# OpenRL-Lab/openrl

Measured on AMD Instinct MI355X. Metric: env-steps/sec (collect+PPO update), 4096-env CartPole-shape, higher is better.
Workload: dtype f32

## Files before the change

### openrl_amd/csrc/orl_mlp.h

```cpp
#pragma once
#include "orl_common.h"

namespace orl {

typedef float f32x4 __attribute__((ext_vector_type(4)));

constexpr int HID = 64;
constexpr int W2S = 68;
constexpr int TILE_B = 16;

#define ORL_MFMA(a, b, c) __builtin_amdgcn_mfma_f32_16x16x4f32((a), (b), (c), 0, 0, 0)
#ifdef ORL_SPLIT_PROBE
#define ORL_IF_FULL(x)
#else
#define ORL_IF_FULL(x) x
#endif

typedef unsigned u32x4 __attribute__((ext_vector_type(4)));
typedef __bf16 bf16x8 __attribute__((ext_vector_type(8)));
typedef float f32x16 __attribute__((ext_vector_type(16)));

#ifndef ORL_WBS
#define ORL_WBS 80
#endif
// ... 244 lines not shown
  return __builtin_bit_cast(unsigned, __builtin_convertvector(f32x2{a, b}, f16x2));
}
__device__ __forceinline__ float rem16_lo(unsigned pk, float x) {
  float r;
  asm("v_fma_mix_f32 %0, %1, -1.0, %2 op_sel_hi:[1,0,0]" : "=v"(r) : "v"(pk), "v"(x));
  return r;
}
__device__ __forceinline__ float rem16_hi(unsigned pk, float x) {
  float r;
  asm("v_fma_mix_f32 %0, %1, -1.0, %2 op_sel:[1,0,0] op_sel_hi:[1,0,0]" : "=v"(r) : "v"(pk), "v"(x));
  return r;
}
__device__ __forceinline__ void split8h(const float (&x)[8], u32x4& hi, u32x4& lo) {
#pragma unroll
  for (int p = 0; p < 4; ++p) {
    const float a = x[2 * p], b = x[2 * p + 1];
    hi[p] = cvt_pk_f16(a, b);
    lo[p] = cvt_pk_f16(rem16_lo(hi[p], a), rem16_hi(hi[p], b));
  }
}
__device__ __forceinline__ f32x4 mfma_f16_16(u32x4 a, u32x4 b, f32x4 c) {
  return __builtin_amdgcn_mfma_f32_16x16x32_f16(__builtin_bit_cast(f16x8, a), __builtin_bit_cast(f16x8, b), c, 0, 0, 0);
}
__device__ __forceinline__ f32x16 mfma_f16_32(u32x4 a, u32x4 b, f32x16 c) {
  return __builtin_amdgcn_mfma_f32_32x32x16_f16(__builtin_bit_cast(f16x8, a), __builtin_bit_cast(f16x8, b), c, 0, 0, 0);
}
__device__ __forceinline__ void split_weight_store2h(unsigned short* __restrict__ img, int o, int k, float w0, float w1) {
  const int m = k >> 4, q = (k >> 2) & 3, r = k & 3, h = m >> 1, sl = (m & 1) * 4 + r;
  const unsigned hi = cvt_pk_f16(w0, w1);
  *(unsigned*)(img + wb_off(0, o, h, q) + sl) = hi;
  *(unsigned*)(img + wb_off(1, o, h, q) + sl) = cvt_pk_f16(rem16_lo(hi, w0), rem16_hi(hi, w1));
}
__device__ __forceinline__ void split_Th(const f32x4 (&in)[4], u32x4 (&xs)[2][2]) {
#pragma unroll
  for (int h = 0; h < 2; ++h) {
    float x[8];
#pragma unroll
    for (int r = 0; r < 4; ++r) { x[r] = in[2 * h][r]; x[4 + r] = in[2 * h + 1][r]; }
    split8h(x, xs[h][0], xs[h][1]);
  }
}
__device__ __forceinline__ void mm64_T_h2(const unsigned short* __restrict__ Wb, const u32x4 (&xs)[2][2], f32x4 (&acc)[4], int j,
                                          int q) {
  u32x4 w[2][2];
#pragma unroll
  for (int p = 0; p < 2; ++p) w[0][p] = *(const u32x4*)(Wb + wb_off(p, j, 0, q));
#pragma unroll
  for (int st = 0; st < 8; ++st) {
    const int h = st >> 2, mo = st & 3;
    if (st < 7) {
      const int h2 = (st + 1) >> 2, mo2 = (st + 1) & 3;
#pragma unroll
      for (int p = 0; p < 2; ++p) w[(st + 1) & 1][p] = *(const u32x4*)(Wb + wb_off(p, 16 * mo2 + j, h2, q));
    }
    const u32x4 wh = w[st & 1][0], wl = w[st & 1][1];
    acc[mo] = mfma_f16_16(wl, xs[h][0], acc[mo]);
    acc[mo] = mfma_f16_16(wh, xs[h][1], acc[mo]);
    acc[mo] = mfma_f16_16(wh, xs[h][0], acc[mo]);
  }
}
__device__ __forceinline__ void mm64_T_h2_tr(const unsigned short* __restrict__ Wb, const u32x4 (&xs)[2][2], f32x4 (&acc)[4],
                                             int j, int q) {
  const unsigned short* base = Wb + (4 * q + (j >> 2)) * WBS + (j & 3) * 8;
  auto frag = [&](int p, int h, int mo) -> u32x4 {
    const unsigned short* a = base + (p * HID + 32 * h) * WBS + (mo >> 1) * 32 + (mo & 1) * 4;
    const u32x2 lo = ds_read_tr16(a), hi = ds_read_tr16(a + 16 * WBS);
    return u32x4{lo[0], lo[1], hi[0], hi[1]};
  };
  u32x4 w[2][2];
#pragma unroll
  for (int p = 0; p < 2; ++p) w[0][p] = frag(p, 0, 0);
#pragma unroll
  for (int st = 0; st < 8; ++st) {
    const int h = st >> 2, mo = st & 3;
    if (st < 7) {
#pragma unroll
      for (int p = 0; p < 2; ++p) w[(st + 1) & 1][p] = frag(p, (st + 1) >> 2, (st + 1) & 3);
    }
    const u32x4 wh = w[st & 1][0], wl = w[st & 1][1];
    acc[mo] = mfma_f16_16(wl, xs[h][0], acc[mo]);
    acc[mo] = mfma_f16_16(wh, xs[h][1], acc[mo]);
    acc[mo] = mfma_f16_16(wh, xs[h][0], acc[mo]);
  }
}
__device__ __forceinline__ float wave_absmax(float v) {
  v = fmaxf(v, u2f(__builtin_amdgcn_update_dpp(0u, f2u(v), 0x121, 0xf, 0xf, false)));
  v = fmaxf(v, u2f(__builtin_amdgcn_update_dpp(0u, f2u(v), 0x122, 0xf, 0xf, false)));
  v = fmaxf(v, u2f(__builtin_amdgcn_update_dpp(0u, f2u(v), 0x124, 0xf, 0xf, false)));
  v = fmaxf(v, u2f(__builtin_amdgcn_update_dpp(0u, f2u(v), 0x128, 0xf, 0xf, false)));
  return row_allmax(v);
}
__device__ __forceinline__ int scale_exponent(float mx) {
  int e = (int)(f2u(mx) >> 23) & 0xff;
  e = e < 20 ? 20 : e;
  return e > 254 ? 254 : e;
}

struct TowerLds {
  int DP, n_out, W1, b1, g1, be1, W2, b2, g2, be2, W3, b3, logstd, W2T, W3P, wsc, total;
  __host__ __device__ TowerLds() {}
  __host__ __device__ TowerLds(int D, int n_out_, bool gaussian, bool with_w2t, bool with_w3p = false,
                               bool split = false) {
    const int w2_floats = split ? TOWER_SPLIT_IMG_FLOATS : HID * W2S;
    DP = (D + 3) & ~3;
    n_out = n_out_;
    const int no4 = (n_out + 3) & ~3;
    int o = 0;
    W1 = o; o += HID * DP;
    b1 = o; o += HID;
    g1 = o; o += HID;
    be1 = o; o += HID;
    W2 = o; o += w2_floats;
    b2 = o; o += HID;
    g2 = o; o += HID;
    be2 = o; o += HID;
    W3 = o; o += with_w3p ? 0 : no4 * HID;
    b3 = o; o += no4;
    logstd = o; o += gaussian ? no4 : 0;
    W2T = o; o += with_w2t ? w2_floats : 0;
    W3P = o; o += with_w3p ? 16 * W2S : 0;
    wsc = o; o += (split && ORL_TOWER_F16) ? 20 : 0;
    total = o;
  }
};

__device__ inline void stage_tower(float* __restrict__ lds, const float* __restrict__ theta, const TowerLayout& tl,
                                   const TowerLds& tw, bool with_w2t, int tid, int nthreads, bool with_w3p = false,
                                   bool split = false, bool fold = false) {
  const int D = tl.D;
  const int no4 = (tl.n_out + 3) & ~3;
  const int n_w3p = with_w3p ? 16 * W2S : 0;
  const int n_w1 = HID * tw.DP;
  const int n_w2 = split ? (HID / 2) * (HID / 2) : HID * HID;
  const int n_w3 = with_w3p ? 0 : no4 * HID;
  const int rows = HID + tl.n_out;
  const int n_fb = fold ? rows * 8 : 0;
  int n_max = n_w3p > n_w1 ? n_w3p : n_w1;
  n_max = n_w2 > n_max ? n_w2 : n_max;
  n_max = n_w3 > n_max ? n_w3 : n_max;
  n_max = n_fb > n_max ? n_fb : n_max;
  n_max = HID > n_max ? HID : n_max;
  unsigned short* b2i = (unsigned short*)(lds + tw.W2);
  unsigned short* b2t = (unsigned short*)(lds + tw.W2T);
  float wscale = 1.f;
  struct Round {
    float p_w, p_g, w1v, vb1, vg1, vbe1, vb2, vg2, vbe2, w00, w01, w10, w11, g0, g1v, w3v, w3g, vb3, vls, fw[8], fbe[8], fb;
  };
  auto load_round = [&](int e, Round& R) {
    R.p_w = 0.f; R.p_g = 1.f;
    const int pc = e / W2S, pi = e - pc * W2S;
    if (e < n_w3p && pc < tl.n_out && pi < HID) {
      R.p_w = theta[tl.oW3 + pc * HID + pi];
      if (fold) R.p_g = theta[tl.og2 + pi];
    }
    R.w1v = 0.f;
    const int w1f = e / tw.DP, w1k = e - w1f * tw.DP;
    if (e < n_w1 && w1k < D) R.w1v = theta[tl.oW1 + w1f * D + w1k];
    R.vb1 = R.vg1 = R.vbe1 = R.vb2 = R.vg2 = R.vbe2 = 0.f;
    if (e < HID) {
      R.vb1 = theta[tl.ob1 + e]; R.vg1 = theta[tl.og1 + e]; R.vbe1 = theta[tl.obe1 + e];
      if (!fold) R.vb2 = theta[tl.ob2 + e];
      R.vg2 = theta[tl.og2 + e]; R.vbe2 = theta[tl.obe2 + e];
    }
    R.w00 = R.w01 = R.w10 = R.w11 = 0.f; R.g0 = R.g1v = 1.f;
    const int bo = split ? 2 * (e >> 5) : (e >> 6), bi = split ? 2 * (e & 31) : (e & 63);
    if (e < n_w2) {
// ... 424 lines not shown
```

### openrl_amd/csrc/orl_ppo_tower.h

```cpp
#pragma once
#include "orl_common.h"
#include "orl_mlp.h"

namespace orl {

#ifndef ORL_USE_SETPRIO
#define ORL_USE_SETPRIO 2
#endif
#if ORL_USE_SETPRIO >= 1
#define ORL_PRIO(x) __builtin_amdgcn_s_setprio(x)
#else
#define ORL_PRIO(x) ((void)0)
#endif
#if ORL_USE_SETPRIO >= 2
#define ORL_PRIO2(x)                                                           \
  do {                                                                         \
    if constexpr (ND == 0 || ORL_USE_SETPRIO >= 3) __builtin_amdgcn_s_setprio(x); \
  } while (0)
#else
#define ORL_PRIO2(x) ((void)0)
#endif

#ifdef ORL_PROF
__device__ unsigned long long g_orl_prof[24];
// ... 49 lines not shown
  int lds_floats;
};

__host__ __device__ inline int ring_chunks(PpoArgs& A, bool compact) {
  const int nch = A.R >> 2;
  if (!compact) { A.c0_beg = 0; A.c0_n = nch; A.c1_beg = nch; return nch; }
  const int DP = (A.net.obs_dim + 3) & ~3;
  const int first_tail = A.net.head_kind == ORL_HEAD_VALUE ? A.o_vp : A.o_act;
  A.c0_beg = A.o_x >> 2;
  int c0_end = ((A.o_x + DP - 1) >> 2) + 1;
  if (c0_end > nch) c0_end = nch;
  A.c0_n = c0_end - A.c0_beg;
  A.c1_beg = first_tail >> 2;
  if (A.c1_beg < c0_end) A.c1_beg = c0_end;
  return A.c0_n + (nch - A.c1_beg);
}

__device__ inline float huber_or_mse(float e, float d, int use_huber, float& de) {
  if (use_huber) {
    const float ae = fabsf(e);
    if (ae <= d) { de = e; return e * e * 0.5f; }
    de = e > 0.f ? d : -d;
    return d * (ae - d * 0.5f);
  }
  de = e;
  return e * e * 0.5f;
}

__device__ inline void store_slab_T(float* __restrict__ slab, const f32x4 (&x)[4], int j, int q) {
#pragma unroll
  for (int m = 0; m < 4; ++m) *(f32x4*)(slab + j * TS + 16 * m + 4 * q) = x[m];
}
__device__ inline void load_slab_T(const float* __restrict__ slab, f32x4 (&x)[4], int j, int q) {
#pragma unroll
  for (int m = 0; m < 4; ++m) x[m] = *(const f32x4*)(slab + j * TS + 16 * m + 4 * q);
}

__device__ inline void ln_bwd_T(f32x4 (&d)[4], const f32x4 (&xhat)[4], float rstd) {
  float s1 = lane_sum16(d), s2 = lane_dot16(d, xhat);
  row_allsum2(s1, s2);
  const float k1 = -s1 * (1.0f / 64.0f) * rstd, k2 = -s2 * (1.0f / 64.0f) * rstd;
#pragma unroll
  for (int m = 0; m < 4; ++m) d[m] = xhat[m] * k2 + (d[m] * rstd + k1);
}

__device__ inline void mm64_T_wt(const float* __restrict__ Ws, const f32x4 (&in)[4], f32x4 (&acc)[4], int j, int q) {
  float a[2][4];
#pragma unroll
  for (int mo = 0; mo < 4; ++mo) a[0][mo] = Ws[(4 * q) * W2S + j + 16 * mo];
#pragma unroll
  for (int k = 0; k < 16; ++k) {
    const int mi = k >> 2, r = k & 3;
    if (k < 15) {
      const float* row = Ws + (16 * ((k + 1) >> 2) + 4 * q + ((k + 1) & 3)) * W2S + j;
#pragma unroll
      for (int mo = 0; mo < 4; ++mo) a[(k + 1) & 1][mo] = row[16 * mo];
    }
#pragma unroll
    for (int mo = 0; mo < 4; ++mo) acc[mo] = ORL_MFMA(a[k & 1][mo], in[mi][r], acc[mo]);
  }
}

template <int HEAD, int NO, int ND, int SP_ = 0>
__device__ __forceinline__ void ppo_tower_body(const PpoArgs& A, const int bid, const int nblk) {
  extern __shared__ __attribute__((aligned(16))) float smem[];
#ifdef ORL_PROF
  const unsigned long long t_entry = __builtin_readcyclecounter();
#endif
  const TowerLayout tl(A.net);
  const RawLayout rl(A.net);
  constexpr bool HMM = NO > 4;
  constexpr bool SP = SP_ >= 2;
  constexpr bool SPT = SP_ == 3;
  constexpr bool SPW = SP_ >= 1;
  const bool w2t = SPT ? false : (ND == 0 || SP || A.use_w2t);
  const TowerLds tw(ND == 0 ? 4 : A.net.obs_dim, NO <= 4 ? 4 : A.net.n_out, HEAD == ORL_HEAD_GAUSSIAN, w2t, HMM, SP);
  const int DP = tw.DP;
  const int D = A.net.obs_dim;
  const int n_out = A.net.n_out;
  constexpr int NOP = HMM ? 16 : ((NO + 3) & ~3);
  const int wave = threadIdx.x >> 6, l = threadIdx.x & 63, j = l & 15, q = l >> 4;
  const int nch = ND == 0 ? (A.R >> 2) : A.c0_n + ((A.R >> 2) - A.c1_beg);
  const int rts = ND == 0 ? ((nch + 3) >> 2) * 256 : nch * 64;
  const int per_wave = 2 * SLAB + 2 * rts + TILE_B * NOP;
  float* wl = smem + tw.total + wave * per_wave;
  float* X1 = wl;
  float* SS = wl + SLAB;
  float* RR = wl + 2 * SLAB;
  float* DH = RR + 2 * rts;

  const float* lw = smem;
  const orl_ppo_hparams hp = A.hp;

  f32x4 G[4][4];
#pragma unroll
  for (int a = 0; a < 4; ++a)
#pragma unroll
    for (int b = 0; b < 4; ++b) G[a][b] = f32x4{0.f, 0.f, 0.f, 0.f};
  f32x16 GS[2][2];
#pragma unroll
  for (int a = 0; a < 2; ++a)
#pragma unroll
    for (int b = 0; b < 2; ++b)
#pragma unroll
      for (int r = 0; r < 16; ++r) GS[a][b][r] = 0.f;
  float a_db2s[2] = {0.f, 0.f};
  constexpr bool W1S = SPW && ND == 1;
  f32x16 G1S[2];
#pragma unroll
  for (int a = 0; a < 2; ++a)
#pragma unroll
    for (int r = 0; r < 16; ++r) G1S[a][r] = 0.f;
  float a_db1s[2] = {0.f, 0.f};
  constexpr int NDA = ND > 0 ? ND : 1;
  f32x4 G1[4][NDA];
#pragma unroll
  for (int a = 0; a < 4; ++a)
#pragma unroll
    for (int b = 0; b < NDA; ++b) G1[a][b] = f32x4{0.f, 0.f, 0.f, 0.f};
  float w1v[4] = {0.f, 0.f, 0.f, 0.f};
  float a_db2 = 0.f, a_db1 = 0.f, a_db3 = 0.f, a_dls = 0.f;
  float a_db3r[NO];
#pragma unroll
  for (int c = 0; c < NO; ++c) a_db3r[c] = 0.f;
  constexpr int NS3 = HMM ? 1 : NO;
  float a_S3[NS3];
#pragma unroll
  for (int c = 0; c < NS3; ++c) a_S3[c] = 0.f;
  f32x4 S3acc[4];
#pragma unroll
  for (int mi = 0; mi < 4; ++mi) S3acc[mi] = f32x4{0.f, 0.f, 0.f, 0.f};
  float st_active = 0.f, st_rows = 0.f, st_loss = 0.f, st_ent = 0.f, st_ratio = 0.f;

  float vn_mean = 0.f, vn_sd = 1.f;
  if (HEAD == ORL_HEAD_VALUE && hp.use_valuenorm && A.vn_state != nullptr) {
    const float deb = fmaxf(A.vn_state[2], 1e-5f);
    vn_mean = A.vn_state[0] / deb;
    const float msq = A.vn_state[1] / deb;
    vn_sd = sqrtf(fmaxf(msq - vn_mean * vn_mean, 1e-2f));
  }

  const int n_tiles = (A.mb + TILE_B - 1) / TILE_B;
  const int nwv = blockDim.x >> 6;
  const int wave_g = bid * nwv + wave;
  const int n_waves = nblk * nwv;

  auto row_of = [&](int t) -> long long {
    const int ii = t * TILE_B + j;
    if (t >= n_tiles || ii >= A.mb) return 0;
    return (A.idx != nullptr) ? A.idx[ii] : (long long)ii;
  };
  auto issue_dma = [&](float* slot, long long row) {
    const float* src = A.records + (size_t)row * A.R;
#pragma unroll 1
    for (int g = 0; 4 * g < nch; ++g) {
      const int c = 4 * g + q;
      const int rc = ND == 0 ? c : (c < A.c0_n ? A.c0_beg + c : A.c1_beg + (c - A.c0_n));
      const unsigned lds_dst = __builtin_amdgcn_readfirstlane(
          (unsigned)(size_t)(__attribute__((address_space(3))) float*)(slot + g * 256));
      if (c < nch) {
        unsigned keep;
        asm volatile("s_mov_b32 %0, m0\n\ts_mov_b32 m0, %2\n\ts_nop 0\n\tglobal_load_lds_dwordx4 %1, off\n\t"
                     "s_mov_b32 m0, %0"
                     : "=&s"(keep)
                     : "v"(src + 4 * rc), "s"(lds_dst)
                     : "memory");
      }
    }
  };
  long long row_next = 0;
  int ring = 0;
  row_next = row_of(wave_g);
  issue_dma(RR, row_next);
  row_next = row_of(wave_g + n_waves);
  stage_tower(smem, A.theta, tl, tw, w2t, threadIdx.x, blockDim.x, HMM, SP, true);
  __syncthreads();
  constexpr bool F16W = SPW && ORL_TOWER_F16;
  constexpr bool F16G = SP && ORL_TOWER_F16;
  const int kw = F16G ? (int)smem[tw.wsc] : 0;
  const float w_scale = F16G ? smem[tw.wsc + 1] : 1.f, ln2_eps = F16G ? smem[tw.wsc + 3] : 1e-5f;
  int LS = 1000;
  int e_run = 0;

#ifdef ORL_PROF
  __shared__ unsigned long long prof_lds[16];
  const bool prof_on = bid == 0 && wave == 0;
  if (prof_on && l < 16) prof_lds[l] = 0ull;
  unsigned long long t_last = __builtin_readcyclecounter();
  const unsigned long long t_loop0 = t_last;
#endif
  for (int tile = wave_g; tile < n_tiles; tile += n_waves) {
    const int i = tile * TILE_B + j;
    const bool valid = i < A.mb;
    const float* RT = RR + ring * rts;
#if !defined(ORL_PROBE_NO_DMA_WAIT)
    if constexpr (ND == 0 && ORL_DMA_WAIT_DEP) asm volatile("s_waitcnt vmcnt(0)" : "+v"(RT));
    else asm volatile("s_waitcnt vmcnt(0)" ::: "memory");
#endif
    const long long row_cur = row_next;
    row_next = row_of(tile + 2 * n_waves);
    issue_dma(RR + (ring ^ 1) * rts, row_cur);
    ring ^= 1;
    const float* RTX = ND == 0 ? RT : RT - 64 * A.c0_beg;
    const float* RTT = ND == 0 ? RT : RT + 64 * (A.c0_n - A.c1_beg);
#define REC(col) RTT[(((col) >> 2) << 6) + (j << 2) + ((col) & 3)]
#define RECX(col) RTX[(((col) >> 2) << 6) + (j << 2) + ((col) & 3)]
#define REC_R(r, col) RTX[(((col) >> 2) << 6) + ((r) << 2) + ((col) & 3)]

    ORL_T(0);
    float rstd1, rstd2;
    unsigned long long relu_mask[16];
    float hd[NO];
    f32x4 hv = f32x4{0.f, 0.f, 0.f, 0.f};
    f32x4 xh2[4];
    {
      f32x4 z[4];
      load_vec_T(lw + tw.b1, q, z);
      if constexpr (ND == 0 || ND > 2) {
        fc1_T(lw + tw.W1, DP, [&](int s) -> float { return RECX(A.o_x + 4 * s + q); }, z, j, q);
      } else {
        constexpr int MAXS = 4 * ND + 1;
        const int nks = DP >> 2;
        float bq[MAXS], aq[MAXS][4];
#pragma unroll
        for (int s = 0; s < MAXS; ++s) {
          const bool on = s < nks;
          bq[s] = on ? RECX(A.o_x + 4 * s + q) : 0.f;
#pragma unroll
          for (int m = 0; m < 4; ++m) aq[s][m] = on ? lw[tw.W1 + (16 * m + j) * DP + 4 * s + q] : 0.f;
        }
#pragma unroll
        for (int s = 0; s < MAXS; ++s) {
          if (s < nks) {
#pragma unroll
            for (int m = 0; m < 4; ++m) z[m] = ORL_MFMA(aq[s][m], bq[s], z[m]);
          }
        }
      }
#pragma unroll
      for (int m = 0; m < 4; ++m)
#pragma unroll
        for (int r = 0; r < 4; ++r) {
          relu_mask[4 * m + r] = __builtin_amdgcn_ballot_w64(z[m][r] > 0.f);
          z[m][r] = fmaxf(z[m][r], 0.f);
        }
      ln_normalize_T(z, rstd1);
      store_slab_T(X1, z, j, q);
      load_vec_T(lw + tw.b2, q, xh2);
      ORL_T(1);
      ORL_PRIO(1);
      if constexpr (F16G) {
        u32x4 xs[2][2];
        split_Th(z, xs);
        mm64_T_h2((const unsigned short*)(lw + tw.W2), xs, xh2, j, q);
      } else if constexpr (SP) {
        u32x4 xs[2][3];
        split_T(z, xs);
        mm64_T_split((const unsigned short*)(lw + tw.W2), xs, xh2, j, q);
      } else {
        mm64_T(lw + tw.W2, z, xh2, j, q);
      }
      ORL_PRIO(0);
      ORL_T(2);
      ln_normalize_T(xh2, rstd2, ln2_eps);
      if constexpr (F16G) rstd2 *= w_scale;
      store_slab_T(SS, xh2, j, q);
#pragma unroll
      for (int m = 0; m < 4; ++m) z[m] = xh2[m];
      if constexpr (HMM) {
        const int no4 = (n_out + 3) & ~3;
        hv = f32x4{0.f, 0.f, 0.f, 0.f};
        if (4 * q < no4) hv = *(const f32x4*)(lw + tw.b3 + 4 * q);
#pragma unroll
        for (int mi = 0; mi < 4; ++mi) {
          const f32x4 a4 = *(const f32x4*)(lw + tw.W3P + j * W2S + 16 * mi + 4 * q);
#pragma unroll
          for (int r = 0; r < 4; ++r) hv = ORL_MFMA(a4[r], z[mi][r], hv);
        }
      } else {
        head_T<NO>(lw + tw.W3, lw + tw.b3, n_out, z, q, hd);
      }
    }

    ORL_T(3);
    float dh[NO];
#pragma unroll
    for (int c = 0; c < NO; ++c) dh[c] = 0.f;
    f32x4 dhv = f32x4{0.f, 0.f, 0.f, 0.f};
    const float active = valid ? REC(A.o_am) : 0.f;
    if constexpr (HMM) {
      const float w = valid ? (hp.use_policy_active_masks ? active : 1.f) : 0.f;
      const float adv = valid ? REC(A.o_adv) : 0.f;
      if (HEAD == ORL_HEAD_CATEGORICAL) {
        float lg[4], mk[4];
        float mx = -3.0e38f;
#pragma unroll
        for (int r = 0; r < 4; ++r) {
          const int c = 4 * q + r;
          mk[r] = (A.K > 0 && valid && c < n_out) ? REC(A.o_mk + c) : 1.f;
          lg[r] = (mk[r] == 0.f) ? -6e4f : hv[r];
          if (c < n_out) mx = fmaxf(mx, lg[r]);
        }
        mx = row_allmax(mx);
        float se = 0.f;
#pragma unroll
        for (int r = 0; r < 4; ++r)
          if (4 * q + r < n_out) se += __expf(lg[r] - mx);
        se = row_allsum(se);
        const float lse = mx + __logf(se);
        const int act = valid ? (int)REC(A.o_act) : 0;
        const float old_lp = valid ? REC(A.o_lp) : 0.f;
        float pk = 0.f, entp = 0.f;
        float p[4];
#pragma unroll
        for (int r = 0; r < 4; ++r) {
          const int c = 4 * q + r;
          p[r] = 0.f;
          if (c < n_out) {
            const float ell = lg[r] - lse;
            p[r] = __expf(ell);
            entp -= p[r] * ell;
            if (c == act) pk = lg[r];
          }
        }
        const float lp = row_allsum(pk) - lse;
        const float ent = row_allsum(entp);
        float ratio = __expf(lp - old_lp);
        const float ratio_raw = ratio;
        float dr_eff = 1.f;
        if (hp.dual_clip_ppo) {
          if (ratio > hp.dual_clip_coeff) { ratio = hp.dual_clip_coeff; dr_eff = 0.f; }
        }
        const float s1 = ratio * adv;
        const float s2 = fminf(fmaxf(ratio, 1.f - hp.clip_param), 1.f + hp.clip_param) * adv;
        float surr = fminf(s1, s2);
        float gl = -((s1 <= s2) ? adv : 0.f) * dr_eff * ratio_raw;
// ... 203 lines not shown
#pragma unroll
      for (int s = 0; s < 4; ++s) {
        const float a = DH[(4 * s + q) * NOP + j];
#pragma unroll
        for (int mi = 0; mi < 4; ++mi) S3acc[mi] = ORL_MFMA(a, SS[(4 * s + q) * TS + 16 * mi + j], S3acc[mi]);
      }
      for (int r = 0; r < TILE_B; ++r) s_db3 += DH[r * NOP + (l & 15)];
      a_db3 += s_db3;
    } else {
      const int f = l;
#if ORL_DB3_ROWLANE
#pragma unroll
      for (int c = 0; c < NO; ++c) a_db3r[c] += q == 0 ? dh[c] : 0.f;
#pragma unroll
      for (int r = 0; r < TILE_B; ++r) {
        const float xh = SS[r * TS + f];
#pragma unroll
        for (int c = 0; c < NO; ++c) a_S3[c < NS3 ? c : 0] += DH[r * NOP + c] * xh;
      }
#else
      float s3[NO];
#pragma unroll
      for (int c = 0; c < NO; ++c) s3[c] = 0.f;
      float s_db3 = 0.f;
      for (int r = 0; r < TILE_B; ++r) {
        const float xh = SS[r * TS + f];
#pragma unroll
        for (int c = 0; c < NO; ++c) s3[c] += DH[r * NOP + c] * xh;
        s_db3 += DH[r * NOP + (f < NO ? f : 0)];
      }
#pragma unroll
      for (int c = 0; c < NO; ++c) a_S3[c < NS3 ? c : 0] += s3[c];
      a_db3 += s_db3;
#endif
    }
    ORL_T(5);
    f32x4 d2[4];
#pragma unroll
    for (int m = 0; m < 4; ++m) d2[m] = f32x4{0.f, 0.f, 0.f, 0.f};
    if constexpr (HMM) {
      const f32x4 dv = dhv;
#pragma unroll
      for (int r = 0; r < 4; ++r)
#pragma unroll
        for (int mo = 0; mo < 4; ++mo)
          d2[mo] = ORL_MFMA(lw[tw.W3P + (4 * q + r) * W2S + 16 * mo + j], dv[r], d2[mo]);
    } else {
#pragma unroll
      for (int c = 0; c < NO; ++c) {
#pragma unroll
        for (int m = 0; m < 4; ++m) {
          const f32x4 w3 = *(const f32x4*)(lw + tw.W3 + c * HID + 16 * m + 4 * q);
          d2[m] = c == 0 ? w3 * dh[0] : w3 * dh[c] + d2[m];
        }
      }
    }
#if ORL_HMM_XH2_RELOAD
    if constexpr ((HMM && ND > 0) || ORL_HMM_XH2_RELOAD == 2) {
      const float* ssr = SS;
      asm volatile("" : "+v"(ssr));
      f32x4 xh2r[4];
      load_slab_T(ssr, xh2r, j, q);
      ln_bwd_T(d2, xh2r, rstd2);
    } else
#endif
    ln_bwd_T(d2, xh2, rstd2);
    int eA = 138;
    if constexpr (F16W) {
      float mx = 0.f;
#pragma unroll
      for (int m = 0; m < 4; ++m) mx = fmaxf(fmaxf(mx, fmaxf(fabsf(d2[m][0]), fabsf(d2[m][1]))), fmaxf(fabsf(d2[m][2]), fabsf(d2[m][3])));
      eA = __builtin_amdgcn_readfirstlane(scale_exponent(wave_absmax(mx)));
#if ORL_TOWER_RUNSCALE
      if (eA > e_run) {
        const int dl = e_run - eA;
#pragma unroll
        for (int a = 0; a < 2; ++a) {
#pragma unroll
          for (int b = 0; b < 2; ++b)
#pragma unroll
            for (int r = 0; r < 16; ++r) GS[a][b][r] = __builtin_ldexpf(GS[a][b][r], dl);
          a_db2s[a] = __builtin_ldexpf(a_db2s[a], dl);
        }
        e_run = eA;
      }
      eA = e_run;
      LS = 138 - e_run;
#endif
#pragma unroll
      for (int m = 0; m < 4; ++m)
#pragma unroll
        for (int r = 0; r < 4; ++r) d2[m][r] = __builtin_ldexpf(d2[m][r], 138 - eA);
#if !ORL_TOWER_RUNSCALE
      const int ls_new = 12 + 138 - eA;
      if (ls_new < LS) {
        const int dl = ls_new - LS;
#pragma unroll
        for (int a = 0; a < 2; ++a) {
#pragma unroll
          for (int b = 0; b < 2; ++b)
#pragma unroll
            for (int r = 0; r < 16; ++r) GS[a][b][r] = __builtin_ldexpf(GS[a][b][r], dl);
          a_db2s[a] = __builtin_ldexpf(a_db2s[a], dl);
        }
        LS = ls_new;
      }
#endif
    }
    wave_lds_fence();
    store_slab_T(SS, d2, j, q);
    wave_lds_fence();
    ORL_T(6);
    if constexpr (SPW) {
      const int c = l & 31, kb = l >> 5;
#if ORL_TOWER_F16
      {
        const int LB = LS - (138 - eA);
        u32x4 fb[2][2];
#pragma unroll
        for (int b = 0; b < 2; ++b) {
          float xb[8];
#pragma unroll
          for (int k = 0; k < 8; ++k) xb[k] = ORL_TOWER_RUNSCALE ? X1[(8 * kb + k) * TS + 32 * b + c] : __builtin_ldexpf(X1[(8 * kb + k) * TS + 32 * b + c], LB);
          split8h(xb, fb[b][0], fb[b][1]);
        }
#pragma unroll
        for (int bo = 0; bo < 2; ++bo) {
          float xa[8];
          u32x4 fa[2];
#pragma unroll
          for (int k = 0; k < 8; ++k) xa[k] = SS[(8 * kb + k) * TS + 32 * bo + c];
          a_db2s[bo] += ORL_TOWER_RUNSCALE ? ((xa[0] + xa[1]) + (xa[2] + xa[3])) + ((xa[4] + xa[5]) + (xa[6] + xa[7]))
                                           : __builtin_ldexpf(((xa[0] + xa[1]) + (xa[2] + xa[3])) + ((xa[4] + xa[5]) + (xa[6] + xa[7])), LB);
          split8h(xa, fa[0], fa[1]);
#pragma unroll
          for (int bi = 0; bi < 2; ++bi) {
            f32x16 g = GS[bo][bi];
            g = mfma_f16_32(fa[1], fb[bi][0], g);
            g = mfma_f16_32(fa[0], fb[bi][1], g);
            g = mfma_f16_32(fa[0], fb[bi][0], g);
            GS[bo][bi] = g;
          }
        }
      }
      if (false) {
#elif ORL_WGRAD_HALVES
      {
        u32x4 fb[2][3];
#pragma unroll
        for (int b = 0; b < 2; ++b) {
          float xb[8];
#pragma unroll
          for (int k = 0; k < 8; ++k) xb[k] = X1[(8 * kb + k) * TS + 32 * b + c];
          split8(xb, fb[b][0], fb[b][1], fb[b][2]);
        }
#pragma unroll
        for (int bo = 0; bo < 2; ++bo) {
          float xa[8];
          u32x4 fa[3];
#pragma unroll
          for (int k = 0; k < 8; ++k) xa[k] = SS[(8 * kb + k) * TS + 32 * bo + c];
          a_db2s[bo] += ((xa[0] + xa[1]) + (xa[2] + xa[3])) + ((xa[4] + xa[5]) + (xa[6] + xa[7]));
          split8(xa, fa[0], fa[1], fa[2]);
#pragma unroll
          for (int bi = 0; bi < 2; ++bi) {
            f32x16 g = GS[bo][bi];
            ORL_IF_FULL(g = mfma_bf16_32(fa[2], fb[bi][0], g);)
            ORL_IF_FULL(g = mfma_bf16_32(fa[0], fb[bi][2], g);)
            ORL_IF_FULL(g = mfma_bf16_32(fa[1], fb[bi][1], g);)
            g = mfma_bf16_32(fa[1], fb[bi][0], g);
            g = mfma_bf16_32(fa[0], fb[bi][1], g);
            g = mfma_bf16_32(fa[0], fb[bi][0], g);
            GS[bo][bi] = g;
          }
        }
      }
      if (false) {
#else
      {
#endif
      u32x4 fa[2][3], fb[2][3];
#pragma unroll
      for (int b = 0; b < 2; ++b) {
        float xa[8], xb[8];
#pragma unroll
        for (int k = 0; k < 8; ++k) {
          xa[k] = SS[(8 * kb + k) * TS + 32 * b + c];
          xb[k] = X1[(8 * kb + k) * TS + 32 * b + c];
        }
        a_db2s[b] += ((xa[0] + xa[1]) + (xa[2] + xa[3])) + ((xa[4] + xa[5]) + (xa[6] + xa[7]));
        split8(xa, fa[b][0], fa[b][1], fa[b][2]);
        split8(xb, fb[b][0], fb[b][1], fb[b][2]);
      }
      ORL_PRIO2(1);
#ifdef ORL_IGLP_WGRAD
      __builtin_amdgcn_iglp_opt(ORL_IGLP_WGRAD);
#endif
#pragma unroll
      for (int bo = 0; bo < 2; ++bo)
#pragma unroll
        for (int bi = 0; bi < 2; ++bi) {
          f32x16 g = GS[bo][bi];
          ORL_IF_FULL(g = mfma_bf16_32(fa[bo][2], fb[bi][0], g);)
          ORL_IF_FULL(g = mfma_bf16_32(fa[bo][0], fb[bi][2], g);)
          ORL_IF_FULL(g = mfma_bf16_32(fa[bo][1], fb[bi][1], g);)
          g = mfma_bf16_32(fa[bo][1], fb[bi][0], g);
          g = mfma_bf16_32(fa[bo][0], fb[bi][1], g);
          g = mfma_bf16_32(fa[bo][0], fb[bi][0], g);
          GS[bo][bi] = g;
        }
      ORL_PRIO2(0);
      }
    } else
    {
      float s_db = 0.f;
      float av[2][4], bv[2][4];
#pragma unroll
      for (int m = 0; m < 4; ++m) {
        av[0][m] = SS[q * TS + 16 * m + j];
        bv[0][m] = X1[q * TS + 16 * m + j];
      }
#pragma unroll
      for (int s = 0; s < 4; ++s) {
        if (s < 3) {
#pragma unroll
          for (int m = 0; m < 4; ++m) {
            av[(s + 1) & 1][m] = SS[(4 * (s + 1) + q) * TS + 16 * m + j];
            bv[(s + 1) & 1][m] = X1[(4 * (s + 1) + q) * TS + 16 * m + j];
          }
        }
#pragma unroll
        for (int mo = 0; mo < 4; ++mo)
#pragma unroll
          for (int mi = 0; mi < 4; ++mi) G[mo][mi] = ORL_MFMA(av[s & 1][mo], bv[s & 1][mi], G[mo][mi]);
      }
      const int f = l;
      for (int r = 0; r < TILE_B; ++r) s_db += SS[r * TS + f];
      a_db2 += s_db;
    }
    ORL_T(7);
    f32x4 d1[4];
#pragma unroll
    for (int m = 0; m < 4; ++m) d1[m] = f32x4{0.f, 0.f, 0.f, 0.f};
    if constexpr (F16G) {
      u32x4 xs[2][2];
      split_Th(d2, xs);
      ORL_PRIO2(1);
      if constexpr (SPT) mm64_T_h2_tr((const unsigned short*)(lw + tw.W2), xs, d1, j, q);
      else mm64_T_h2((const unsigned short*)(lw + tw.W2T), xs, d1, j, q);
      ORL_PRIO2(0);
    } else if constexpr (SP) {
      u32x4 xs[2][3];
      split_T(d2, xs);
      ORL_PRIO2(1);
      if constexpr (SPT) mm64_T_split_tr((const unsigned short*)(lw + tw.W2), xs, d1, j, q);
      else mm64_T_split((const unsigned short*)(lw + tw.W2T), xs, d1, j, q);
      ORL_PRIO2(0);
    } else {
      if (w2t) mm64_T(lw + tw.W2T, d2, d1, j, q);
      else mm64_T_wt(lw + tw.W2, d2, d1, j, q);
    }
    ORL_T(8);
    {
      f32x4 xh1[4];
      load_slab_T(X1, xh1, j, q);
      ln_bwd_T(d1, xh1, F16W ? __builtin_ldexpf(rstd1, eA - 138 - kw) : rstd1);
    }
#pragma unroll
    for (int m = 0; m < 4; ++m)
#pragma unroll
      for (int r = 0; r < 4; ++r)
        d1[m][r] = __builtin_amdgcn_inverse_ballot_w64(relu_mask[4 * m + r]) ? d1[m][r] : 0.f;
    wave_lds_fence();
    store_slab_T(SS, d1, j, q);
    wave_lds_fence();
    ORL_T(9);
    if constexpr (W1S) {
      const int c = l & 31, kb = l >> 5;
      const int colx = A.o_x + (c < DP ? c : DP - 1);
      const float* xcol = RTX + ((colx >> 2) << 6) + (colx & 3);
      float xv8[8];
#pragma unroll
      for (int k = 0; k < 8; ++k) xv8[k] = xcol[(8 * kb + k) << 2];
      u32x4 fx[3];
      split8(xv8, fx[0], fx[1], fx[2]);
#pragma unroll
      for (int b = 0; b < 2; ++b) {
        float xa[8];
#pragma unroll
        for (int k = 0; k < 8; ++k) xa[k] = SS[(8 * kb + k) * TS + 32 * b + c];
        a_db1s[b] += ((xa[0] + xa[1]) + (xa[2] + xa[3])) + ((xa[4] + xa[5]) + (xa[6] + xa[7]));
        u32x4 fa[3];
        split8(xa, fa[0], fa[1], fa[2]);
        f32x16 g = G1S[b];
        ORL_IF_FULL(g = mfma_bf16_32(fa[2], fx[0], g);)
        ORL_IF_FULL(g = mfma_bf16_32(fa[0], fx[2], g);)
        ORL_IF_FULL(g = mfma_bf16_32(fa[1], fx[1], g);)
        g = mfma_bf16_32(fa[1], fx[0], g);
        g = mfma_bf16_32(fa[0], fx[1], g);
        g = mfma_bf16_32(fa[0], fx[0], g);
        G1S[b] = g;
      }
    } else {
      const int f = l;
      float s_db = 0.f;
      if (ND == 0) {
        f32x4 w4 = f32x4{w1v[0], w1v[1], w1v[2], w1v[3]};
        typedef float f32x2 __attribute__((ext_vector_type(2)));
        f32x2 sd2 = f32x2{0.f, 0.f};
#pragma unroll
        for (int r = 0; r < TILE_B; r += 2) {
          const f32x2 dz = f32x2{SS[r * TS + f], SS[(r + 1) * TS + f]};
          const f32x4 x0 = *(const f32x4*)(&REC_R(r, A.o_x));
          const f32x4 x1 = *(const f32x4*)(&REC_R(r + 1, A.o_x));
          sd2 += dz;
          w4 = x0 * dz[0] + w4;
          w4 = x1 * dz[1] + w4;
        }
        s_db += sd2[0] + sd2[1];
        w1v[0] = w4[0]; w1v[1] = w4[1]; w1v[2] = w4[2]; w1v[3] = w4[3];
      } else {
        const int n_rem = D - 16 * ND;
        if (n_rem > 0) {
#pragma unroll
          for (int r = 0; r < TILE_B; ++r) {
            const float dzv = SS[r * TS + f];
            s_db += dzv;
#pragma unroll
            for (int k = 0; k < 4; ++k) w1v[k] += dzv * REC_R(r, A.o_x + 16 * ND + k);
          }
        } else {
          for (int r = 0; r < TILE_B; ++r) s_db += SS[r * TS + f];
        }
#pragma unroll
        for (int s = 0; s < 4; ++s) {
          float av[4], bv[NDA];
#pragma unroll
          for (int m = 0; m < 4; ++m) av[m] = SS[(4 * s + q) * TS + 16 * m + j];
#pragma unroll
          for (int mk = 0; mk < NDA; ++mk) bv[mk] = (16 * mk + j < D) ? REC_R(4 * s + q, A.o_x + 16 * mk + j) : 0.f;
#pragma unroll
          for (int mf = 0; mf < 4; ++mf)
#pragma unroll
            for (int mk = 0; mk < NDA; ++mk) G1[mf][mk] = ORL_MFMA(av[mf], bv[mk], G1[mf][mk]);
        }
      }
      a_db1 += s_db;
    }
    wave_lds_fence();
    ORL_T(10);
  }
#ifdef ORL_PROF
  if (prof_on && l < 12) atomicAdd(&g_orl_prof[l], prof_lds[l]);
  if (prof_on && l == 12) atomicAdd(&g_orl_prof[12], 1ull);
  if (prof_on && l == 13)
    atomicAdd(&g_orl_prof[13], (unsigned long long)((n_tiles - wave_g + n_waves - 1) / n_waves));
  if (prof_on && l == 14) atomicAdd(&g_orl_prof[14], t_loop0 - t_entry);
  const unsigned long long t_loop1 = __builtin_readcyclecounter();
#endif
#undef REC
#undef RECX
#undef REC_R

  if constexpr (F16W) {
#pragma unroll
    for (int a = 0; a < 2; ++a) {
#pragma unroll
      for (int b = 0; b < 2; ++b)
#pragma unroll
        for (int r = 0; r < 16; ++r) GS[a][b][r] = __builtin_ldexpf(GS[a][b][r], -LS);
      a_db2s[a] = __builtin_ldexpf(a_db2s[a], -LS);
    }
  }
  asm volatile("s_waitcnt vmcnt(0)" ::: "memory");
#ifdef ORL_PROF
  if (prof_on && l == 16) atomicAdd(&g_orl_prof[16], __builtin_readcyclecounter() - t_loop1);
#endif
  __syncthreads();
#ifdef ORL_PROF
  if (prof_on && l == 17) atomicAdd(&g_orl_prof[17], __builtin_readcyclecounter() - t_loop1);
#endif
  const int PW = rl.total + ORL_N_STATS;
  const int lds_have = A.lds_floats > 0 ? A.lds_floats : tw.total + nwv * per_wave;
  constexpr int NREG_MAX = 8;
#ifndef ORL_EPI_FRAG
#define ORL_EPI_FRAG 1
#endif
  constexpr int GN = HID * HID;
  const bool frag_g = ORL_EPI_FRAG && SPW && ND == 0 && nwv <= NREG_MAX && lds_have >= nwv * GN + (PW - GN);
  const int PWI = frag_g ? PW - GN : PW;
  const int IOFF = frag_g ? GN : 0;
  float* gimg = smem;
  float* img0 = smem + (frag_g ? nwv * GN : 0);
  int NREG = (lds_have - (frag_g ? nwv * GN : 0)) / PWI;
  NREG = NREG > nwv ? nwv : NREG < 1 ? 1 : NREG;
  NREG = NREG > NREG_MAX ? NREG_MAX : NREG;
  while (nwv % NREG) --NREG;
  for (int e = threadIdx.x; e < NREG * ORL_N_STATS; e += blockDim.x)
    img0[(size_t)(e / ORL_N_STATS) * PWI + rl.total - IOFF + (e % ORL_N_STATS)] = 0.f;
  if constexpr (SPW) {
    if (frag_g) {
      float* gw = gimg + (size_t)wave * GN + l * 4;
#pragma unroll
      for (int bo = 0; bo < 2; ++bo)
#pragma unroll
        for (int bi = 0; bi < 2; ++bi)
#pragma unroll
          for (int rq = 0; rq < 4; ++rq)
            *(f32x4*)(gw + ((bo * 2 + bi) * 4 + rq) * 256) = f32x4{GS[bo][bi][4 * rq], GS[bo][bi][4 * rq + 1],
                                                                   GS[bo][bi][4 * rq + 2], GS[bo][bi][4 * rq + 3]};
    }
  }
  __syncthreads();
  st_active = wave_sum_dpp(st_active); st_rows = wave_sum_dpp(st_rows); st_loss = wave_sum_dpp(st_loss);
  st_ent = wave_sum_dpp(st_ent); st_ratio = wave_sum_dpp(st_ratio);
#if ORL_DB3_ROWLANE
  if constexpr (!HMM) {
#pragma unroll
    for (int c = 0; c < NO; ++c) {
      const float tot = wave_sum_dpp(a_db3r[c]);
      if (l == c) a_db3 = tot;
    }
  }
#endif
  float* acc = img0 + (size_t)(wave % NREG) * PWI - IOFF;
  for (int p = 0; p < nwv / NREG; ++p) {
    if (wave / NREG == p) {
      const bool first = p == 0;
      auto put = [&](int idx, float v) { acc[idx] = first ? v : acc[idx] + v; };
      const int f = l;
      if constexpr (SPW) {
        auto g_idx = [&](int bo, int bi, int r) {
          return rl.oG + (32 * bo + (r & 3) + 8 * (r >> 2) + 4 * (l >> 5)) * HID + 32 * bi + (l & 31);
        };
        if (frag_g) {
        } else if (first) {
#pragma unroll
          for (int bo = 0; bo < 2; ++bo)
#pragma unroll
            for (int bi = 0; bi < 2; ++bi)
#pragma unroll
              for (int r = 0; r < 16; ++r) acc[g_idx(bo, bi, r)] = GS[bo][bi][r];
        } else {
          float old[2][2][16];
#pragma unroll
          for (int bo = 0; bo < 2; ++bo)
#pragma unroll
            for (int bi = 0; bi < 2; ++bi)
#pragma unroll
              for (int r = 0; r < 16; ++r) old[bo][bi][r] = acc[g_idx(bo, bi, r)];
#pragma unroll
          for (int bo = 0; bo < 2; ++bo)
#pragma unroll
            for (int bi = 0; bi < 2; ++bi)
#pragma unroll
              for (int r = 0; r < 16; ++r) acc[g_idx(bo, bi, r)] = old[bo][bi][r] + GS[bo][bi][r];
        }
        const float d0 = xor32_sum(a_db2s[0]), d1s = xor32_sum(a_db2s[1]);
        if (l < 32) {
          put(rl.odb2 + l, d0);
          put(rl.odb2 + 32 + l, d1s);
        }
      } else {
        auto g_idx = [&](int mo, int mi, int r) { return rl.oG + (16 * mo + 4 * q + r) * HID + 16 * mi + j; };
        if (first) {
#pragma unroll
          for (int mo = 0; mo < 4; ++mo)
#pragma unroll
            for (int mi = 0; mi < 4; ++mi)
#pragma unroll
              for (int r = 0; r < 4; ++r) acc[g_idx(mo, mi, r)] = G[mo][mi][r];
        } else {
          float old[4][4][4];
#pragma unroll
          for (int mo = 0; mo < 4; ++mo)
#pragma unroll
            for (int mi = 0; mi < 4; ++mi)
#pragma unroll
              for (int r = 0; r < 4; ++r) old[mo][mi][r] = acc[g_idx(mo, mi, r)];
#pragma unroll
          for (int mo = 0; mo < 4; ++mo)
#pragma unroll
            for (int mi = 0; mi < 4; ++mi)
#pragma unroll
              for (int r = 0; r < 4; ++r) acc[g_idx(mo, mi, r)] = old[mo][mi][r] + G[mo][mi][r];
        }
        put(rl.odb2 + f, a_db2);
      }
      if constexpr (W1S) {
        const float e0 = xor32_sum(a_db1s[0]), e1 = xor32_sum(a_db1s[1]);
        if (l < 32) {
          put(rl.odb1 + l, e0);
          put(rl.odb1 + 32 + l, e1);
        }
      } else {
        put(rl.odb1 + f, a_db1);
      }
      if constexpr (HMM) {
        auto s_idx = [&](int mi, int r) { return rl.oS3 + (4 * q + r) * HID + 16 * mi + j; };
        float old[4][4];
        if (!first) {
#pragma unroll
          for (int mi = 0; mi < 4; ++mi)
#pragma unroll
            for (int r = 0; r < 4; ++r) old[mi][r] = 4 * q + r < n_out ? acc[s_idx(mi, r)] : 0.f;
        }
#pragma unroll
        for (int mi = 0; mi < 4; ++mi)
#pragma unroll
          for (int r = 0; r < 4; ++r)
            if (4 * q + r < n_out) acc[s_idx(mi, r)] = first ? S3acc[mi][r] : old[mi][r] + S3acc[mi][r];
      } else {
#pragma unroll
        for (int c = 0; c < NO; ++c)
          if (c < n_out) put(rl.oS3 + c * HID + f, a_S3[c < NS3 ? c : 0]);
      }
      if (f < n_out) put(rl.odb3 + f, a_db3);
      if (HEAD == ORL_HEAD_GAUSSIAN && f < n_out) put(rl.odlogstd + f, a_dls);
      if constexpr (W1S) {
        if ((l & 31) < D) {
          auto w_idx = [&](int bo, int r) { return rl.odW1 + (32 * bo + (r & 3) + 8 * (r >> 2) + 4 * (l >> 5)) * D + (l & 31); };
          float old[2][16];
          if (!first) {
#pragma unroll
            for (int bo = 0; bo < 2; ++bo)
#pragma unroll
              for (int r = 0; r < 16; ++r) old[bo][r] = acc[w_idx(bo, r)];
          }
#pragma unroll
          for (int bo = 0; bo < 2; ++bo)
#pragma unroll
            for (int r = 0; r < 16; ++r) acc[w_idx(bo, r)] = first ? G1S[bo][r] : old[bo][r] + G1S[bo][r];
        }
      } else if (ND == 0) {
#pragma unroll
        for (int k = 0; k < 4; ++k)
          if (k < D) put(rl.odW1 + f * D + k, w1v[k]);
      } else {
#pragma unroll
        for (int mf = 0; mf < 4; ++mf)
#pragma unroll
          for (int mk = 0; mk < NDA; ++mk)
#pragma unroll
            for (int r = 0; r < 4; ++r) {
              const int kk = 16 * mk + j;
              if (kk < D) put(rl.odW1 + (16 * mf + 4 * q + r) * D + kk, G1[mf][mk][r]);
            }
#pragma unroll
        for (int k = 0; k < 4; ++k)
          if (16 * ND + k < D) put(rl.odW1 + f * D + 16 * ND + k, w1v[k]);
      }
      if (l == 0) {
        put(rl.total + ST_ACTIVE_SUM, st_active);
        put(rl.total + ST_ROWS, st_rows);
        if (HEAD == ORL_HEAD_VALUE) put(rl.total + ST_VLOSS_SUM, st_loss);
        else {
          put(rl.total + ST_PLOSS_SUM, st_loss);
          put(rl.total + ST_ENT_SUM, st_ent);
          put(rl.total + ST_RATIO_SUM, st_ratio);
        }
      }
    }
    __syncthreads();
  }
#ifdef ORL_PROF
  if (prof_on && l == 18) atomicAdd(&g_orl_prof[18], __builtin_readcyclecounter() - t_loop1);
#endif
  float* out = A.partials + (size_t)bid * PW;
  if (frag_g) {
    for (int k = threadIdx.x; k < GN / 4; k += blockDim.x) {
      const int Rq = k >> 6, ln = k & 63;
      f32x4 v[NREG_MAX];
#pragma unroll
      for (int w = 0; w < NREG_MAX; ++w)
        v[w] = w < nwv ? *(const f32x4*)(gimg + (size_t)w * GN + Rq * 256 + ln * 4) : f32x4{0.f, 0.f, 0.f, 0.f};
      f32x4 t = v[0];
#pragma unroll
      for (int w = 1; w < NREG_MAX; ++w) t += v[w];
      const int o0 = 32 * (Rq >> 3) + 8 * (Rq & 3) + 4 * (ln >> 5), i = 32 * ((Rq >> 2) & 1) + (ln & 31);
#pragma unroll
      for (int rr = 0; rr < 4; ++rr) out[(o0 + rr) * HID + i] = t[rr];
    }
  }
#pragma unroll 2
  for (int e = IOFF + threadIdx.x; e < PW; e += blockDim.x) {
    float v[NREG_MAX];
#pragma unroll
    for (int g = 0; g < NREG_MAX; ++g) v[g] = g < NREG ? img0[(size_t)g * PWI + e - IOFF] : 0.f;
    float t = v[0];
#pragma unroll
    for (int g = 1; g < NREG_MAX; ++g) t += v[g];
    out[e] = t;
  }
#ifdef ORL_PROF
  if (prof_on && l == 15) atomicAdd(&g_orl_prof[15], __builtin_readcyclecounter() - t_loop1);
#endif
}

template <int HEAD, int NO, int ND>
__global__ __launch_bounds__(512, 2) void ppo_tower_kernel(PpoArgs A) {
  ppo_tower_body<HEAD, NO, ND>(A, (int)blockIdx.x, (int)gridDim.x);
}

#ifndef ORL_PAIR_WAVES
#define ORL_PAIR_WAVES 8
#endif
template <int HEADP, int NOP_, int ND, int SP = 0>
__global__ __launch_bounds__(64 * ORL_PAIR_WAVES, (ORL_PAIR_WAVES + 3) / 4) void ppo_tower_pair_kernel(PpoArgs P, PpoArgs Cc, int gp) {
  if ((int)blockIdx.x < gp) ppo_tower_body<HEADP, NOP_, ND, SP>(P, (int)blockIdx.x, gp);
  else ppo_tower_body<ORL_HEAD_VALUE, 1, ND, SP>(Cc, (int)blockIdx.x - gp, (int)gridDim.x - gp);
}

inline size_t tower_lds_floats(const orl_net_desc& net, int R, int nop, int waves, bool gaussian, bool w2t = true,
                               bool split = false, int ring_nch = -1) {
  const TowerLds tw(net.obs_dim, net.n_out, gaussian, w2t, nop == 16, split);
  const RawLayout rl(net);
  if (ring_nch < 0) ring_nch = R >> 2;
  const int rts = net.obs_dim <= 4 ? (((R >> 2) + 3) >> 2) * 256 : ring_nch * 64;
  const size_t per_wave = 2 * SLAB + 2 * rts + TILE_B * nop;
  size_t fl = (size_t)tw.total + (size_t)waves * per_wave;
  const size_t pw = (size_t)rl.total + ORL_N_STATS;
  const size_t need_acc = pw;
  const size_t all_waves = (size_t)waves * pw;
  if (fl < all_waves && all_waves * sizeof(float) <= 160 * 1024) fl = all_waves;
  return fl > need_acc ? fl : need_acc;
}

}
```

Measured before the change: 258.5 million.

## Store W2-grad operands as swizzled f16 tiles and accumulate db2 in registers

In the f16 run-scale tower path, the d2 gradient and, in the SPT variant, the X1 activations are stored to LDS as pre-split hi/lo f16 tiles with an XOR swizzle. The W2 gradient MFMA then reads them with transposed LDS loads instead of rebuilding fragments from f32 slabs and splitting them on every step. The db2 bias gradient is accumulated in per-lane registers and reduced once with DPP at the end, and the split d2 fragments are reused for the backward matmul. This adds an extra per-wave LDS tile and more registers, which may lower occupancy or change LDS sizing.

```diff
diff --git a/openrl_amd/csrc/orl_mlp.h b/openrl_amd/csrc/orl_mlp.h
--- a/openrl_amd/csrc/orl_mlp.h
+++ b/openrl_amd/csrc/orl_mlp.h
@@ -350,6 +350,28 @@
     acc[mo] = mfma_f16_16(wh, xs[h][1], acc[mo]);
     acc[mo] = mfma_f16_16(wh, xs[h][0], acc[mo]);
   }
+}
+constexpr int H16_PART = TILE_B * HID;
+constexpr int H16_TILE_FLOATS = 2 * H16_PART / 2;
+__device__ __forceinline__ int h16_swz(int row) { return ((row & 2) << 1) | ((row & 1) << 1) | ((row >> 2) & 1); }
+__device__ __forceinline__ void store_tile_h16(unsigned short* __restrict__ tile, const u32x4 (&xs)[2][2], int j, int q) {
+#pragma unroll
+  for (int h = 0; h < 2; ++h)
+#pragma unroll
+    for (int p = 0; p < 2; ++p) *(u32x4*)(tile + p * H16_PART + j * HID + 8 * ((4 * h + q) ^ h16_swz(j))) = xs[h][p];
+}
+__device__ __forceinline__ u32x4 load_frag_h16(const unsigned short* __restrict__ tile, int p, int b, int j, int q) {
+  const int r0 = 8 * (q >> 1) + (j >> 2), r1 = r0 + 4, un = 4 * b + (j & 3);
+  const u32x2 lo = ds_read_tr16(tile + p * H16_PART + r0 * HID + 8 * (un ^ h16_swz(r0)) + 4 * (q & 1));
+  const u32x2 hi = ds_read_tr16(tile + p * H16_PART + r1 * HID + 8 * (un ^ h16_swz(r1)) + 4 * (q & 1));
+  return u32x4{lo[0], lo[1], hi[0], hi[1]};
+}
+__device__ __forceinline__ float row16_sum_dpp(float v) {
+  v += u2f(__builtin_amdgcn_update_dpp(0u, f2u(v), 0x121, 0xf, 0xf, false));
+  v += u2f(__builtin_amdgcn_update_dpp(0u, f2u(v), 0x122, 0xf, 0xf, false));
+  v += u2f(__builtin_amdgcn_update_dpp(0u, f2u(v), 0x124, 0xf, 0xf, false));
+  v += u2f(__builtin_amdgcn_update_dpp(0u, f2u(v), 0x128, 0xf, 0xf, false));
+  return v;
 }
 __device__ __forceinline__ float wave_absmax(float v) {
   v = fmaxf(v, u2f(__builtin_amdgcn_update_dpp(0u, f2u(v), 0x121, 0xf, 0xf, false)));
diff --git a/openrl_amd/csrc/orl_ppo_tower.h b/openrl_amd/csrc/orl_ppo_tower.h
--- a/openrl_amd/csrc/orl_ppo_tower.h
+++ b/openrl_amd/csrc/orl_ppo_tower.h
@@ -155,12 +155,16 @@
   const int wave = threadIdx.x >> 6, l = threadIdx.x & 63, j = l & 15, q = l >> 4;
   const int nch = ND == 0 ? (A.R >> 2) : A.c0_n + ((A.R >> 2) - A.c1_beg);
   const int rts = ND == 0 ? ((nch + 3) >> 2) * 256 : nch * 64;
-  const int per_wave = 2 * SLAB + 2 * rts + TILE_B * NOP;
+  constexpr bool DZH = SPW && ORL_TOWER_F16 && ORL_TOWER_RUNSCALE && ND == 0;
+  constexpr bool X1H = DZH && SPT;
+  const int per_wave = 2 * SLAB + 2 * rts + TILE_B * NOP + (X1H ? H16_TILE_FLOATS : 0);
   float* wl = smem + tw.total + wave * per_wave;
   float* X1 = wl;
   float* SS = wl + SLAB;
   float* RR = wl + 2 * SLAB;
   float* DH = RR + 2 * rts;
+  unsigned short* SSh = (unsigned short*)SS;
+  unsigned short* X1h = (unsigned short*)(DH + TILE_B * NOP);
 
   const float* lw = smem;
   const orl_ppo_hparams hp = A.hp;
@@ -178,6 +182,9 @@
 #pragma unroll
       for (int r = 0; r < 16; ++r) GS[a][b][r] = 0.f;
   float a_db2s[2] = {0.f, 0.f};
+  f32x4 db2p[4];
+#pragma unroll
+  for (int m = 0; m < 4; ++m) db2p[m] = f32x4{0.f, 0.f, 0.f, 0.f};
   constexpr bool W1S = SPW && ND == 1;
   f32x16 G1S[2];
 #pragma unroll
@@ -325,6 +332,7 @@
       if constexpr (F16G) {
         u32x4 xs[2][2];
         split_Th(z, xs);
+        if constexpr (X1H) store_tile_h16(X1h, xs, j, q);
         mm64_T_h2((const unsigned short*)(lw + tw.W2), xs, xh2, j, q);
       } else if constexpr (SP) {
         u32x4 xs[2][3];
@@ -694,6 +702,12 @@
             for (int r = 0; r < 16; ++r) GS[a][b][r] = __builtin_ldexpf(GS[a][b][r], dl);
           a_db2s[a] = __builtin_ldexpf(a_db2s[a], dl);
         }
+        if constexpr (DZH) {
+#pragma unroll
+          for (int m = 0; m < 4; ++m)
+#pragma unroll
+            for (int r = 0; r < 4; ++r) db2p[m][r] = __builtin_ldexpf(db2p[m][r], dl);
+        }
         e_run = eA;
       }
       eA = e_run;
@@ -719,14 +733,48 @@
       }
 #endif
     }
+    u32x4 xs2[2][2];
     wave_lds_fence();
-    store_slab_T(SS, d2, j, q);
+    if constexpr (DZH) {
+#pragma unroll
+      for (int m = 0; m < 4; ++m) db2p[m] += d2[m];
+      split_Th(d2, xs2);
+      store_tile_h16(SSh, xs2, j, q);
+    } else {
+      store_slab_T(SS, d2, j, q);
+    }
     wave_lds_fence();
     ORL_T(6);
     if constexpr (SPW) {
       const int c = l & 31, kb = l >> 5;
 #if ORL_TOWER_F16
-      {
+      if constexpr (DZH) {
+        u32x4 fb[2][2];
+#pragma unroll
+        for (int b = 0; b < 2; ++b) {
+          if constexpr (X1H) {
+            fb[b][0] = load_frag_h16(X1h, 0, b, j, q);
+            fb[b][1] = load_frag_h16(X1h, 1, b, j, q);
+          } else {
+            float xb[8];
+#pragma unroll
+            for (int k = 0; k < 8; ++k) xb[k] = X1[(8 * kb + k) * TS + 32 * b + c];
+            split8h(xb, fb[b][0], fb[b][1]);
+          }
+        }
+#pragma unroll
+        for (int bo = 0; bo < 2; ++bo) {
+          const u32x4 fa0 = load_frag_h16(SSh, 0, bo, j, q), fa1 = load_frag_h16(SSh, 1, bo, j, q);
+#pragma unroll
+          for (int bi = 0; bi < 2; ++bi) {
+            f32x16 g = GS[bo][bi];
+            g = mfma_f16_32(fa1, fb[bi][0], g);
+            g = mfma_f16_32(fa0, fb[bi][1], g);
+            g = mfma_f16_32(fa0, fb[bi][0], g);
+            GS[bo][bi] = g;
+          }
+        }
+      } else {
         const int LB = LS - (138 - eA);
         u32x4 fb[2][2];
 #pragma unroll
@@ -855,11 +903,10 @@
 #pragma unroll
     for (int m = 0; m < 4; ++m) d1[m] = f32x4{0.f, 0.f, 0.f, 0.f};
     if constexpr (F16G) {
-      u32x4 xs[2][2];
-      split_Th(d2, xs);
+      if constexpr (!DZH) split_Th(d2, xs2);
       ORL_PRIO2(1);
-      if constexpr (SPT) mm64_T_h2_tr((const unsigned short*)(lw + tw.W2), xs, d1, j, q);
-      else mm64_T_h2((const unsigned short*)(lw + tw.W2T), xs, d1, j, q);
+      if constexpr (SPT) mm64_T_h2_tr((const unsigned short*)(lw + tw.W2), xs2, d1, j, q);
+      else mm64_T_h2((const unsigned short*)(lw + tw.W2T), xs2, d1, j, q);
       ORL_PRIO2(0);
     } else if constexpr (SP) {
       u32x4 xs[2][3];
@@ -982,6 +1029,12 @@
 #pragma unroll
         for (int r = 0; r < 16; ++r) GS[a][b][r] = __builtin_ldexpf(GS[a][b][r], -LS);
       a_db2s[a] = __builtin_ldexpf(a_db2s[a], -LS);
+    }
+    if constexpr (DZH) {
+#pragma unroll
+      for (int m = 0; m < 4; ++m)
+#pragma unroll
+        for (int r = 0; r < 4; ++r) db2p[m][r] = row16_sum_dpp(__builtin_ldexpf(db2p[m][r], -LS));
     }
   }
   asm volatile("s_waitcnt vmcnt(0)" ::: "memory");
@@ -1068,10 +1121,19 @@
 #pragma unroll
               for (int r = 0; r < 16; ++r) acc[g_idx(bo, bi, r)] = old[bo][bi][r] + GS[bo][bi][r];
         }
-        const float d0 = xor32_sum(a_db2s[0]), d1s = xor32_sum(a_db2s[1]);
-        if (l < 32) {
-          put(rl.odb2 + l, d0);
-          put(rl.odb2 + 32 + l, d1s);
+        if constexpr (DZH) {
+          if (j == 0) {
+#pragma unroll
+            for (int m = 0; m < 4; ++m)
+#pragma unroll
+              for (int r = 0; r < 4; ++r) put(rl.odb2 + 16 * m + 4 * q + r, db2p[m][r]);
+          }
+        } else {
+          const float d0 = xor32_sum(a_db2s[0]), d1s = xor32_sum(a_db2s[1]);
+          if (l < 32) {
+            put(rl.odb2 + l, d0);
+            put(rl.odb2 + 32 + l, d1s);
+          }
         }
       } else {
         auto g_idx = [&](int mo, int mi, int r) { return rl.oG + (16 * mo + 4 * q + r) * HID + 16 * mi + j; };
@@ -1229,7 +1291,8 @@
   const RawLayout rl(net);
   if (ring_nch < 0) ring_nch = R >> 2;
   const int rts = net.obs_dim <= 4 ? (((R >> 2) + 3) >> 2) * 256 : ring_nch * 64;
-  const size_t per_wave = 2 * SLAB + 2 * rts + TILE_B * nop;
+  const bool x1h = ORL_TOWER_F16 && ORL_TOWER_RUNSCALE && split && !w2t && net.obs_dim <= 4;
+  const size_t per_wave = 2 * SLAB + 2 * rts + TILE_B * nop + (x1h ? H16_TILE_FLOATS : 0);
   size_t fl = (size_t)tw.total + (size_t)waves * per_wave;
   const size_t pw = (size_t)rl.total + ORL_N_STATS;
   const size_t need_acc = pw;
```

Measured after the change: 251.9 million. 0.974x the previous value.
